# UnchartedWhispers/Distributed-Data-Parallel-Experiment

Measured on AMD Instinct MI355X. Metric: samples_per_sec_whole_node, higher is better.
Workload: dtype bf16

## Files before the change

### csrc/include/ddpx_wgrad_sgd.h

```cpp
#pragma once

#include <cstdlib>

#include "ddpx_mx.h"
#include "ddpx_pipe.h"

namespace ddpx {
namespace wsgd {

constexpr int BM = 64, BN = 128;
constexpr int A_SUB = BM * 64 * 2, B_SUB = BN * 64 * 2, SLOT = A_SUB + B_SUB;
constexpr int VPT = BM * BN / 4 / 256;
constexpr int kStampSlots = 256;

template <int STAGES>
struct Cfg {
  static_assert(STAGES == 3 || STAGES == 4, "ring depth");
  static constexpr int ALD = STAGES >= 4 ? BN : BN + 4;
  static constexpr int ACC_BYTES = BM * ALD * 4;
  static constexpr int LDS_BYTES = STAGES * SLOT + 2 * ACC_BYTES;
  static_assert(LDS_BYTES <= 160 * 1024, "LDS");
};

template <int STAGES, bool FP8, int NSW, bool NORD, int NMW, int PROBE = 0>
__global__ void __launch_bounds__(64 * NMW + 64 * NSW) wgrad_sgd_ws_kernel(pipe::Params p0, pipe::Params p1, int nt1) {
  constexpr int ALD = Cfg<STAGES>::ALD, ACC_BYTES = Cfg<STAGES>::ACC_BYTES;
  constexpr int LDS_BYTES = Cfg<STAGES>::LDS_BYTES;
  static_assert(NMW == 4 || NMW == 8, "math waves");
  static_assert(PROBE == 0 || PROBE == 3 || PROBE == 4, "probe");
  constexpr int WN = NMW / 2;
  constexpr int FM = 2, FN = BN / WN / 16;
  constexpr int LPW = (BM + BN) / (8 * NMW);
  __shared__ __attribute__((aligned(1024))) char smem[LDS_BYTES];
  float* const accb = reinterpret_cast<float*>(smem + STAGES * SLOT);

  const int tid = threadIdx.x;
  const int lane = tid & 63;
  const int wave = __builtin_amdgcn_readfirstlane(tid >> 6);
  const int tiles_m0 = p0.M / BM, tiles_m1 = p1.M / BM;
  const int nt0 = tiles_m0 * (p0.N / BN);
  const int ntiles = nt0 + nt1;
  const int nt = (ntiles - (int)blockIdx.x + (int)gridDim.x - 1) / (int)gridDim.x;
  const int nk = p0.K / 64;
  auto tile_origin = [&](int i, int& m0, int& n0) -> int {
    int g = (int)blockIdx.x + i * (int)gridDim.x;
    const int sel = g >= nt0;
    if (sel) g -= nt0;
    if constexpr (NORD) {
      const int tn = (sel ? p1.N : p0.N) / BN;
      m0 = (g / tn) * BM;
      n0 = (g % tn) * BN;
    } else {
      const int tm = sel ? tiles_m1 : tiles_m0;
      m0 = (g % tm) * BM;
      n0 = (g / tm) * BN;
    }
    return sel;
  };
  const pipe::Params& p = p0;
  long long* const stp = (p0.stamp && (tid == 0 || tid == 64 * NMW))
                             ? p0.stamp + ((size_t)blockIdx.x * 2 + (wave < NMW ? 0 : 1)) * kStampSlots
                             : nullptr;
  int nstamp = 1;
  auto mark = [&]() {
    if (stp) {
      stp[nstamp < kStampSlots - 1 ? nstamp : kStampSlots - 2] = (long long)__builtin_amdgcn_s_memrealtime();
      ++nstamp;
    }
  };
  if (stp) stp[0] = (long long)__builtin_amdgcn_s_memrealtime();

  if (wave < NMW) {
    const int wm = wave / WN, wn = wave % WN;
    const __amdgpu_buffer_rsrc_t ra0 = __builtin_amdgcn_make_buffer_rsrc((void*)p0.A, 0, p0.a_bytes, 0x00020000);
    const __amdgpu_buffer_rsrc_t rb0 = __builtin_amdgcn_make_buffer_rsrc((void*)p0.B, 0, p0.b_bytes, 0x00020000);
    const __amdgpu_buffer_rsrc_t ra1 = __builtin_amdgcn_make_buffer_rsrc((void*)p1.A, 0, p1.a_bytes, 0x00020000);
    const __amdgpu_buffer_rsrc_t rb1 = __builtin_amdgcn_make_buffer_rsrc((void*)p1.B, 0, p1.b_bytes, 0x00020000);
    const int G = nt * nk;
    int iss_i = -1, iss_kt = nk - 1, iss_m0 = 0, iss_n0 = 0, iss_sel = 0;
    auto issue = [&](int g) {
      if constexpr (PROBE == 4) return;
      if (++iss_kt >= nk) {
        iss_kt = 0;
        iss_sel = tile_origin(++iss_i, iss_m0, iss_n0);
      }
      const int m0 = iss_m0, n0 = iss_n0, sel = iss_sel, kt = iss_kt;
      const __amdgpu_buffer_rsrc_t ra = sel ? ra1 : ra0, rb = sel ? rb1 : rb0;
      const int lda = sel ? p1.lda : p0.lda, ldb = sel ? p1.ldb : p0.ldb;
      const int Mg = sel ? p1.M : p0.M, Ng = sel ? p1.N : p0.N;
      char* slot = smem + (g % STAGES) * SLOT;
      pipe::stage_tile<BM, false, pipe::MODE_PLAIN, NMW>(ra, slot, p.conv, lda, m0, Mg, kt * 64, p.K, wave, lane);
      pipe::stage_tile<BN, false, pipe::MODE_PLAIN, NMW>(rb, slot + A_SUB, p.conv, ldb, n0, Ng, kt * 64, p.K, wave,
                                                         lane);
    };
#pragma unroll
    for (int s = 0; s < STAGES - 1; ++s)
      if (s < G) issue(s);
    for (int i = 0; i <= nt; ++i) {
      if (i == nt) {
        for (int t = 0; t < nk; ++t) {
          mark();
          __builtin_amdgcn_s_barrier();
        }
      } else {
        f32x4 acc[FM][FN];
#pragma unroll
        for (int a = 0; a < FM; ++a)
#pragma unroll
          for (int b = 0; b < FN; ++b) acc[a][b] = (f32x4){0.f, 0.f, 0.f, 0.f};
        for (int t = 0; t < nk; ++t) {
          const int g = i * nk + t;
          const int ahead = min(STAGES - 2, G - 1 - g);
          if (STAGES >= 4 && ahead >= 2) pipe::wait_vmcnt<2 * LPW>();
          else if (ahead >= 1) pipe::wait_vmcnt<LPW>();
          else pipe::wait_vmcnt<0>();
          mark();
          __builtin_amdgcn_s_barrier();
          asm volatile("" ::: "memory");
          if (g + STAGES - 1 < G) issue(g + STAGES - 1);
          const char* sa = smem + (g % STAGES) * SLOT;
          const char* sb = sa + A_SUB;
#pragma unroll
          for (int kk = 0; kk < (PROBE == 4 ? 0 : 64); kk += 32) {
            bf16x8 af[FM], bfr[FN];
            pipe::load_frags<BM, false, FM, BN, false, FN>(sa, wm * 32, sb, wn * (BN / WN), kk, lane, af, bfr);
#pragma unroll
            for (int a = 0; a < FM; ++a)
#pragma unroll
              for (int b = 0; b < FN; ++b)
                acc[a][b] = __builtin_amdgcn_mfma_f32_16x16x32_bf16(af[a], bfr[b], acc[a][b], 0, 0, 0);
          }
        }
        float* T = accb + (i & 1) * (ACC_BYTES / 4);
        const int mr = wm * 32 + 4 * (lane >> 4), nc = wn * (BN / WN) + (lane & 15);
#pragma unroll
        for (int a = 0; a < FM; ++a)
#pragma unroll
          for (int b = 0; b < FN; ++b)
#pragma unroll
            for (int r = 0; r < 4; ++r) T[(mr + a * 16 + r) * ALD + nc + b * 16] = acc[a][b][r] * p.alpha;
      }
      asm volatile("s_waitcnt lgkmcnt(0)" ::: "memory");
      mark();
      __builtin_amdgcn_s_barrier();
    }
    if (stp) stp[kStampSlots - 1] = (long long)__builtin_amdgcn_s_memrealtime();
  } else {
    constexpr int DIST = 4;
    constexpr int SV = BM * BN / 4 / (NSW * 64);
    constexpr int KPU = VPT / SV;
    constexpr int RSTEP = NSW * 2;
    static_assert(SV % DIST == 0 && VPT % SV == 0, "ring");
    const int st = tid - 64 * NMW;
    const int row0 = st >> 5, col = 4 * (st & 31);
    const float lr = *p.sgd.lr;
    const float mom = p.sgd.mom, wd = p.sgd.wd;
    const bool has_mom = mom != 0.f;
    f32x4 rp[DIST], rm[DIST];
    float* const P0 = p0.sgd.p;
    float* const P1 = p1.sgd.p;
    float* const M0 = has_mom ? p0.sgd.buf : p0.sgd.p;
    float* const M1 = has_mom ? p1.sgd.buf : p1.sgd.p;
    unsigned short* const S0 = p0.sgd.shadow;
    unsigned short* const S1 = p1.sgd.shadow;
    unsigned char* const Q0 = p0.sgd.q8;
    unsigned char* const Q1 = p1.sgd.q8;
    unsigned char* const E0 = p0.sgd.s8;
    unsigned char* const E1 = p1.sgd.s8;
    unsigned char* const QT0 = p0.sgd.q8t;
    unsigned char* const QT1 = p1.sgd.q8t;
    unsigned char* const ET0 = p0.sgd.s8t;
    unsigned char* const ET1 = p1.sgd.s8t;
    const bool qt_on = FP8 && NSW == 8 && (QT0 != nullptr || QT1 != nullptr);
    unsigned qt_e0 = 0;
    const int ldc0 = p0.ldc, ldc1 = p1.ldc;
    auto vec_off = [&](int j, int v, int& sel) -> size_t {
      int m0, n0;
      sel = tile_origin(j, m0, n0);
      return (size_t)(m0 + row0 + RSTEP * v) * (sel ? ldc1 : ldc0) + n0 + col;
    };
    auto load_vec = [&](int j, int v, f32x4& pv, f32x4& mv) {
      int sel;
      const size_t off = vec_off(j, v, sel);
      pv = __builtin_nontemporal_load(reinterpret_cast<const f32x4*>((sel ? P1 : P0) + off));
      mv = __builtin_nontemporal_load(reinterpret_cast<const f32x4*>((sel ? M1 : M0) + off));
    };
    auto grad_vec = [&](const float* T, int v) -> f32x4 {
      return *reinterpret_cast<const f32x4*>(T + (row0 + RSTEP * v) * ALD + col);
    };
    auto update_vec_g = [&](int j, int v, const f32x4 g, f32x4& pv, f32x4& mv, float* stage) {
      int sel;
      const size_t off = vec_off(j, v, sel);
      f32x4 po, bo;
#pragma unroll
      for (int q = 0; q < 4; ++q) {
        float d = fmaf(wd, pv[q], g[q]);
        if (has_mom) d = fmaf(mom, mv[q], d);
        po[q] = fmaf(-lr, d, pv[q]);
        bo[q] = has_mom ? d : po[q];
      }
      if (stage) *reinterpret_cast<f32x4*>(stage) = po;
      const u32x2 sh = (u32x2){pack_bf2(po[0], po[1]), pack_bf2(po[2], po[3])};
      __builtin_nontemporal_store(po, reinterpret_cast<f32x4*>((sel ? P1 : P0) + off));
      __builtin_nontemporal_store(bo, reinterpret_cast<f32x4*>((sel ? M1 : M0) + off));
      *reinterpret_cast<u32x2*>((sel ? S1 : S0) + off) = sh;
      if constexpr (FP8) {
        unsigned e8;
        const unsigned q = mx::e4m3_group8(po, &e8);
        *reinterpret_cast<unsigned*>((sel ? Q1 : Q0) + off) = q;
        const unsigned e1 = (unsigned)__builtin_amdgcn_update_dpp(0, (int)e8, 0x128, 0xF, 0xF, false);
        if ((lane & 15) == 0)
          *reinterpret_cast<unsigned short*>((sel ? E1 : E0) + (off >> 5)) = (unsigned short)(e8 | (e1 << 8));
      }
      const int vn = v + DIST;
      const bool same = vn < SV, next = !same && j + 1 < nt;
      load_vec(same ? j : (next ? j + 1 : j), same ? vn : (next ? vn - SV : v), pv, mv);
    };
    auto update_vec = [&](int j, int v, const float* T, f32x4& pv, f32x4& mv) {
      if constexpr (FP8 && NSW == 8) {
        if (qt_on) {
          float* slot = const_cast<float*>(T) + (row0 + RSTEP * v) * ALD + col;
          const f32x4 g = *reinterpret_cast<const f32x4*>(slot);
          update_vec_g(j, v, g, pv, mv, slot);
          asm volatile("s_waitcnt lgkmcnt(0)" ::: "memory");
          return;
        }
      }
      update_vec_g(j, v, grad_vec(T, v), pv, mv, nullptr);
    };
    auto quant_t = [&](int j, int b, const float* T) {
      int m0, n0;
      const int sel = tile_origin(j, m0, n0);
      unsigned char* const qd = sel ? QT1 : QT0;
      if (!qd) return;
      const int c = st >> 2, sub = st & 3;
      float v[8];
      float am = 0.f;
#pragma unroll
      for (int r = 0; r < 8; ++r) {
        v[r] = bf2f(f2bf(T[(32 * b + 8 * sub + r) * ALD + c]));
        am = fmaxf(am, fabsf(v[r]));
      }
      am = fmaxf(am, __builtin_bit_cast(float, __builtin_amdgcn_update_dpp(0, __builtin_bit_cast(int, am), 0xB1, 0xF, 0xF, false)));
      am = fmaxf(am, __builtin_bit_cast(float, __builtin_amdgcn_update_dpp(0, __builtin_bit_cast(int, am), 0x4E, 0xF, 0xF, false)));
      const int e = mx::block_exp(am, mx::kMaxE4M3);
      const float inv = ldexpf(1.f, -e);
      const unsigned lo = mx::quant4(v[0], v[1], v[2], v[3], inv, mx::kMaxE4M3, false);
      const unsigned hi = mx::quant4(v[4], v[5], v[6], v[7], inv, mx::kMaxE4M3, false);
      const int Mg = sel ? p1.M : p0.M;
      *reinterpret_cast<u32x2*>(qd + (size_t)(n0 + c) * Mg + m0 + 32 * b + 8 * sub) = (u32x2){lo, hi};
      unsigned char* const ed = sel ? ET1 : ET0;
      if (sub == 0 && ed) {
        if (b == 0) {
          qt_e0 = (unsigned)(e + 127);
        } else {
          *reinterpret_cast<unsigned short*>(ed + (size_t)(n0 + c) * (Mg / 32) + m0 / 32) =
              (unsigned short)(qt_e0 | ((unsigned)(e + 127) << 8));
        }
      }
    };
#pragma unroll
    for (int v = 0; v < DIST; ++v)
      if constexpr (PROBE != 3) load_vec(0, v, rp[v], rm[v]);
    for (int t = 0; t < nk; ++t) {
      mark();
      __builtin_amdgcn_s_barrier();
    }
    mark();
    __builtin_amdgcn_s_barrier();
    constexpr int TPI = SV / DIST;
    auto trip = [&](int r) {
      const int i = 1 + r / TPI, t = (r % TPI) * DIST;
      const float* T = accb + ((i - 1) & 1) * (ACC_BYTES / 4);
#pragma unroll
      for (int u = 0; u < DIST; ++u) {
        mark();
        __builtin_amdgcn_s_barrier();
        __builtin_amdgcn_sched_barrier(0);
        if constexpr (PROBE != 3) update_vec(i - 1, t + u, T, rp[u], rm[u]);
        __builtin_amdgcn_sched_barrier(0);
#pragma unroll
        for (int k = 1; k < KPU; ++k) {
          mark();
          __builtin_amdgcn_s_barrier();
        }
        if constexpr (FP8 && NSW == 8) {
          if (qt_on && (t + u) % 2 == 1) {
            quant_t(i - 1, (t + u) / 2, T);
            asm volatile("s_waitcnt lgkmcnt(0)" ::: "memory");
          }
        }
      }
      if (r % TPI == TPI - 1) {
        asm volatile("s_waitcnt lgkmcnt(0)" ::: "memory");
        mark();
        __builtin_amdgcn_s_barrier();
      }
    };
    trip(0);
#pragma unroll 1
    for (int r = 1; r < TPI * nt; ++r) trip(r);
    if (stp) stp[kStampSlots - 1] = (long long)__builtin_amdgcn_s_memrealtime();
  }
}

static inline bool eligible(const pipe::Params& p, bool ak, bool bk) {
  return !ak && !bk && p.M % BM == 0 && p.N % BN == 0 && p.K == 64 * VPT && (p.ldc & 3) == 0 && p.sgd.p &&
         p.sgd.lr && (p.sgd.mom == 0.f || p.sgd.buf) && p.sgd.shadow && (!p.sgd.q8 || (p.sgd.s8 && (p.ldc & 127) == 0 && !((uintptr_t)p.sgd.q8 & 3) && !((uintptr_t)p.sgd.s8 & 3))) &&
         (!p.sgd.q8t || (p.sgd.q8 && !((uintptr_t)p.sgd.q8t & 7) && !((uintptr_t)p.sgd.s8t & 1)));
}

struct Variant {
  int stages;
  bool fp8;
  int nsw;
  bool nord;
  int nmw;
  int probe;
};

static inline int env_digit(const char* name) {
  const char* e = getenv(name);
  return e && e[0] >= '0' && e[0] <= '9' ? e[0] - '0' : -1;
}

static inline Variant select_variant(long long ntiles, int num_cus, bool fp8, bool qt) {
  static const int env_stages = env_digit("DDPX_WSGD_STAGES"), env_nsw = env_digit("DDPX_WSGD_STREAM_WAVES");
  static const int env_nmw = env_digit("DDPX_WSGD_MATH_WAVES");
  static const int env_probe = [] {
    const char* e = getenv("DDPX_WSGD_XTRA");
    return e ? atoi(e) : 0;
  }();
  static const bool env_nord = [] {
    const char* e = getenv("DDPX_WSGD_ORDER");
    return !(e && e[0] == 'm');
  }();
  const bool large = ntiles >= 64LL * num_cus;
  Variant v;
  v.stages = (env_stages == 3 || env_stages == 4) ? env_stages : (large ? 4 : 3);
  v.fp8 = fp8;
  v.nsw = qt ? 8 : (env_nsw == 4 || env_nsw == 8) ? env_nsw : (large ? 8 : 4);
  v.nord = env_nord;
  v.nmw = (env_nmw != 4 && v.nsw == 4 && v.nord) ? 8 : 4;
  const bool toy = !fp8 && v.stages == 3 && v.nsw == 4 && v.nord;
  v.probe = (toy && (env_probe == 3 || env_probe == 4)) ? env_probe : 0;
  return v;
}

using Kernel = void (*)(pipe::Params, pipe::Params, int);

template <int STAGES, bool FP8>
static inline Kernel layout_kernel(const Variant& v) {
  if (v.nmw == 8) return wgrad_sgd_ws_kernel<STAGES, FP8, 4, true, 8>;
  if (v.nsw == 8) return v.nord ? wgrad_sgd_ws_kernel<STAGES, FP8, 8, true, 4>
                                : wgrad_sgd_ws_kernel<STAGES, FP8, 8, false, 4>;
  return v.nord ? wgrad_sgd_ws_kernel<STAGES, FP8, 4, true, 4> : wgrad_sgd_ws_kernel<STAGES, FP8, 4, false, 4>;
}

static inline Kernel kernel_of(const Variant& v) {
  if (v.probe == 3)
    return v.nmw == 8 ? wgrad_sgd_ws_kernel<3, false, 4, true, 8, 3> : wgrad_sgd_ws_kernel<3, false, 4, true, 4, 3>;
  if (v.probe == 4)
    return v.nmw == 8 ? wgrad_sgd_ws_kernel<3, false, 4, true, 8, 4> : wgrad_sgd_ws_kernel<3, false, 4, true, 4, 4>;
  if (v.stages == 4) return v.fp8 ? layout_kernel<4, true>(v) : layout_kernel<4, false>(v);
  return v.fp8 ? layout_kernel<3, true>(v) : layout_kernel<3, false>(v);
}

static inline hipError_t launch_variant(const pipe::Params& p0, const pipe::Params& p1, int nt1, bool qt, int num_cus,
                                        hipStream_t s) {
  const int ntiles = (p0.M / BM) * (p0.N / BN) + nt1;
  const int grid = ntiles < num_cus ? ntiles : num_cus;
  const Variant v = select_variant(ntiles, num_cus, p0.sgd.q8 != nullptr, qt);
  hipLaunchKernelGGL(kernel_of(v), dim3(grid), dim3(64 * (v.nmw + v.nsw)), 0, s, p0, p1, nt1);
  return hipGetLastError();
}

static inline hipError_t launch(const pipe::Params& p, int num_cus, hipStream_t s) {
  return launch_variant(p, p, 0, false, num_cus, s);
}

static inline bool pair_compatible(const pipe::Params& a, const pipe::Params& b) {
  return a.K == b.K && a.alpha == b.alpha && a.sgd.lr == b.sgd.lr && a.sgd.mom == b.sgd.mom && a.sgd.wd == b.sgd.wd;
}

static inline hipError_t launch_pair(const pipe::Params& p0, const pipe::Params& p1, int num_cus, hipStream_t s) {
  if ((p0.sgd.q8 != nullptr) != (p1.sgd.q8 != nullptr)) return hipErrorInvalidValue;
  const bool qt = p0.sgd.q8t != nullptr || p1.sgd.q8t != nullptr;
  if (qt && !p0.sgd.q8) return hipErrorInvalidValue;
  return launch_variant(p0, p1, (p1.M / BM) * (p1.N / BN), qt, num_cus, s);
}

}
}
```

### csrc/kernels/gemm_pipe.hip

```cpp
#include <cstdlib>

#include "ddpx_gemm_dispatch.h"
#include "ddpx_pipe.h"
#include "ddpx_wgrad_sgd.h"

namespace ddpx {
namespace pipe {

static int pick(int M, int N, int K, bool ak, bool bk) {
  auto tiles = [&](int bm, int bn) { return ((M + bm - 1) / bm) * ((N + bn - 1) / bn); };
  if (!ak && !bk) return tiles(64, 128) >= 512 ? 5 : 7;
  if (tiles(128, 128) >= 512 && K >= 2048) return 21;
  return 12;
}

static int plan(int M, int N, int K, bool ak, bool bk, int epi, int* cfg) {
  *cfg = pick(M, N, K, ak, bk);
  static const int sk_cfg = [] {
    const char* e = getenv("DDPX_SPLITK");
    return e ? atoi(e) : 0;
  }();
  static const int sk_max = [] {
    const char* e = getenv("DDPX_SPLITK_MAX");
    return e ? atoi(e) : 2;
  }();
  if (sk_cfg <= 0 || !ak || epi == EPI_SGD || epi == EPI_BNSTAT_BF16 || K < 1024) return 1;
  int bm, bn;
  tile_of(sk_cfg, &bm, &bn);
  const int target = (sk_cfg == 5 || sk_cfg == 6 || sk_cfg == 7) ? 512 : 256;
  const int t = ((M + bm - 1) / bm) * ((N + bn - 1) / bn);
  if (t * 4 >= target * 3) return 1;
  int s = target / t;
  if (s > sk_max) s = sk_max;
  while (s > 1 && (K / 64) / s < 8) --s;
  if (s < 2) return 1;
  *cfg = sk_cfg;
  return s;
}

}
}

using namespace ddpx;

static long long* g_stamp = nullptr;

DDPX_API void ddpx_gemm_set_stamps(long long* buf) { g_stamp = buf; }

DDPX_API int ddpx_gemm_pipe_tiles_m(int M, int N, int K, int a_kcontig, int b_kcontig, int tile_cfg) {
  int cfg = tile_cfg;
  if (cfg < 0) pipe::plan(M, N, K, a_kcontig, b_kcontig, pipe::EPI_BF16, &cfg);
  int bm, bn;
  pipe::tile_of(cfg, &bm, &bn);
  return (M + bm - 1) / bm;
}

DDPX_API void ddpx_gemm_tile_dims(int cfg, int* bm, int* bn) { pipe::tile_of(cfg, bm, bn); }

DDPX_API int ddpx_gemm_pipe_plan(int M, int N, int K, int a_kcontig, int b_kcontig, int epi, int* cfg,
                                 long long* slab_floats, int* tickets) {
  const int s = pipe::plan(M, N, K, a_kcontig, b_kcontig, epi, cfg);
  int bm, bn;
  pipe::tile_of(*cfg, &bm, &bn);
  const long long tiles = (long long)((M + bm - 1) / bm) * ((N + bn - 1) / bn);
  *slab_floats = s > 1 ? (long long)s * tiles * bm * bn : 0;
  *tickets = s > 1 ? (int)tiles : 0;
  return s;
}

DDPX_API int ddpx_gemm_pipe(const void* A, const void* B, void* C, const float* bias, const void* aux, float* colsum,
                            int M, int N, int K, int lda, int ldb, int ldc, int ldaux, int a_kcontig, int b_kcontig,
                            int epi, int accumulate, float alpha, int tile_cfg, float* sgd_p, float* sgd_buf,
                            void* sgd_shadow, const float* sgd_lr, float sgd_mom, float sgd_wd, int splits,
                            float* slab, long long slab_floats, int* tcnt, void* cs_out, int cs_flags,
                            int* cs_tcnt, hipStream_t stream) {
  if (M <= 0 || N <= 0 || K <= 0) return 0;
  if (a_kcontig ? (K % 8 || lda % 8) : (M % 8 || lda % 8)) return -1;
  if (b_kcontig ? (K % 8 || ldb % 8) : (N % 8 || ldb % 8)) return -2;
  if ((reinterpret_cast<uintptr_t>(A) | reinterpret_cast<uintptr_t>(B)) & 15) return -3;
  const size_t a_bytes = (size_t)(a_kcontig ? (size_t)(M - 1) * lda + K : (size_t)(K - 1) * lda + M) * 2;
  const size_t b_bytes = (size_t)(b_kcontig ? (size_t)(N - 1) * ldb + K : (size_t)(K - 1) * ldb + N) * 2;
  if (a_bytes >= 0x80000000ull || b_bytes >= 0x80000000ull) return -4;
  pipe::Params p{(const unsigned short*)A, (const unsigned short*)B, C, bias, (const unsigned short*)aux, colsum,
                 M, N, K, lda, ldb, ldc, ldaux, epi, accumulate, alpha, (unsigned)a_bytes, (unsigned)b_bytes,
                 SgdArgs{sgd_p, sgd_buf, (unsigned short*)sgd_shadow, sgd_lr, sgd_mom, sgd_wd},
                 pipe::make_geom(0, 0, 0, 0), 0, 0, 0, nullptr, 0u, nullptr, cs_out, cs_flags, cs_tcnt};
  p.stamp = g_stamp;
  if (cs_tcnt && (!colsum || epi == pipe::EPI_SGD || epi == pipe::EPI_BNSTAT_BF16 || (!cs_out && !sgd_p) ||
                  (sgd_p && !sgd_lr)))
    return -10;
  if (epi == pipe::EPI_SGD && (!sgd_p || !sgd_lr || (sgd_mom != 0.f && !sgd_buf))) return -5;
  static const int sgd_plain = [] {
    const char* e = getenv("DDPX_SGD_PLAIN");
    return e && e[0] == '1' ? 1 : 0;
  }();
  p.sgd_plain = sgd_plain;
  int cfg = tile_cfg >= 0 ? tile_cfg : pipe::pick(M, N, K, a_kcontig, b_kcontig);
  if (cs_tcnt && pipe::eight_wave(cfg)) return -11;
  if (cfg >= 16 && cfg <= 20 && (epi == pipe::EPI_SGD || epi == pipe::EPI_BNSTAT_BF16)) return -12;
  if (splits > 1) {
    if (epi == pipe::EPI_SGD || epi == pipe::EPI_BNSTAT_BF16 || !slab || !tcnt || tile_cfg < 0 || !a_kcontig)
      return -7;
    int bm, bn;
    pipe::tile_of(cfg, &bm, &bn);
    const long long tiles = (long long)((M + bm - 1) / bm) * ((N + bn - 1) / bn);
    if (slab_floats < (long long)splits * tiles * bm * bn || slab_floats * 4 >= 0x80000000ll) return -8;
    int klen = (K + splits - 1) / splits;
    klen = (klen + 63) / 64 * 64;
    if ((K + klen - 1) / klen != splits) return -9;
    p.klen = klen;
    p.slab = slab;
    p.slab_bytes = (unsigned)(slab_floats * 4);
    p.tcnt = tcnt;
  }
  if (tile_cfg < 0 && !a_kcontig && !b_kcontig && epi != pipe::EPI_SGD && !colsum &&
      ((M + 255) / 256) * ((N + 255) / 256) >= 128)
    cfg = 13;
  static const int wgrad_ws = [] {
    const char* e = getenv("DDPX_WGRAD_WS");
    return e && e[0] == '0' ? 0 : 1;
  }();
  if (epi == pipe::EPI_SGD && wgrad_ws && tile_cfg < 0 && splits <= 1 && wsgd::eligible(p, a_kcontig, b_kcontig)) {
    static const int cus = [] {
      int dev = 0, n = 0;
      if (hipGetDevice(&dev) != hipSuccess ||
          hipDeviceGetAttribute(&n, hipDeviceAttributeMultiprocessorCount, dev) != hipSuccess || n <= 0)
        n = 256;
      return n;
    }();
    return (int)wsgd::launch(p, cus, stream);
  }
  hipError_t e;
  if (splits > 1) {
    e = b_kcontig ? pipe::dispatch_sk_kk(p, cfg, splits, stream) : pipe::dispatch_sk_kn(p, cfg, splits, stream);
    return (int)e;
  }
  const int S = 1;
  if (a_kcontig && b_kcontig) e = pipe::dispatch_kk(p, cfg, S, stream);
  else if (a_kcontig) e = pipe::dispatch_kn(p, cfg, S, stream);
  else if (b_kcontig) e = pipe::dispatch_mk(p, cfg, S, stream);
  else e = pipe::dispatch_mn(p, cfg, S, stream);
  return (int)e;
}

DDPX_API int ddpx_wgrad_sgd_pair_t(const void* A0, const void* B0, int M0, int N0, int lda0, int ldb0, int ldc0,
                                   float* p0, float* buf0, void* sh0, void* q80, void* s80, void* q8t0, void* s8t0,
                                   const void* A1, const void* B1, int M1, int N1, int lda1, int ldb1, int ldc1,
                                   float* p1, float* buf1, void* sh1, void* q81, void* s81, void* q8t1, void* s8t1,
                                   int K, const float* lr, float mom, float wd, hipStream_t stream) {
  auto make = [&](const void* A, const void* B, int M, int N, int lda, int ldb, int ldc, float* pp, float* buf,
                  void* sh, void* q8, void* s8, void* q8t, void* s8t) {
    const size_t a_bytes = ((size_t)(K - 1) * lda + M) * 2, b_bytes = ((size_t)(K - 1) * ldb + N) * 2;
    return pipe::Params{(const unsigned short*)A, (const unsigned short*)B, pp, nullptr, nullptr, nullptr,
                        M, N, K, lda, ldb, ldc, 0, pipe::EPI_SGD, 0, 1.f, (unsigned)a_bytes, (unsigned)b_bytes,
                        SgdArgs{pp, buf, (unsigned short*)sh, lr, mom, wd, (unsigned char*)q8, (unsigned char*)s8,
                                (unsigned char*)q8t, (unsigned char*)s8t},
                        pipe::make_geom(0, 0, 0, 0), 0, 0, 0, nullptr, 0u, nullptr, nullptr, 0, nullptr};
  };
  if (K <= 0 || lda0 % 8 || ldb0 % 8 || lda1 % 8 || ldb1 % 8 || M0 % 8 || N0 % 8 || M1 % 8 || N1 % 8) return -20;
  if (((uintptr_t)A0 | (uintptr_t)B0 | (uintptr_t)A1 | (uintptr_t)B1) & 15) return -20;
  if ((q8t0 || q8t1) && (!q80 || !q81)) return -20;
  pipe::Params q0 = make(A0, B0, M0, N0, lda0, ldb0, ldc0, p0, buf0, sh0, q80, s80, q8t0, s8t0);
  const pipe::Params q1 = make(A1, B1, M1, N1, lda1, ldb1, ldc1, p1, buf1, sh1, q81, s81, q8t1, s8t1);
  q0.stamp = g_stamp;
  if ((size_t)q0.a_bytes != ((size_t)(K - 1) * lda0 + M0) * 2 || (size_t)q1.b_bytes != ((size_t)(K - 1) * ldb1 + N1) * 2)
    return -20;
  if (!wsgd::eligible(q0, false, false) || !wsgd::eligible(q1, false, false) || !wsgd::pair_compatible(q0, q1))
    return -20;
  if ((q80 != nullptr) != (q81 != nullptr)) return -20;
  int dev = 0, cus = 0;
  if (hipGetDevice(&dev) != hipSuccess ||
      hipDeviceGetAttribute(&cus, hipDeviceAttributeMultiprocessorCount, dev) != hipSuccess || cus <= 0)
    cus = 256;
  return (int)wsgd::launch_pair(q0, q1, cus, stream);
}

DDPX_API int ddpx_wgrad_sgd_pair(const void* A0, const void* B0, int M0, int N0, int lda0, int ldb0, int ldc0,
                                 float* p0, float* buf0, void* sh0, void* q80, void* s80, const void* A1,
                                 const void* B1, int M1, int N1, int lda1, int ldb1, int ldc1, float* p1, float* buf1,
                                 void* sh1, void* q81, void* s81, int K, const float* lr, float mom, float wd,
                                 hipStream_t stream) {
  return ddpx_wgrad_sgd_pair_t(A0, B0, M0, N0, lda0, ldb0, ldc0, p0, buf0, sh0, q80, s80, nullptr, nullptr, A1, B1,
                               M1, N1, lda1, ldb1, ldc1, p1, buf1, sh1, q81, s81, nullptr, nullptr, K, lr, mom, wd,
                               stream);
}
```

### ddpx/ops/gemm.py

```python
from __future__ import annotations

import torch

from ..runtime import native


EPI_F32 = 0
EPI_BF16 = 1
EPI_BIAS_BF16 = 2
EPI_BIAS_RELU_BF16 = 3
EPI_BIAS_F32 = 4
EPI_RELUMASK_BF16 = 5
EPI_SGD = 6

_OUT_DTYPE = {
    EPI_F32: torch.float32,
    EPI_BF16: torch.bfloat16,
    EPI_BIAS_BF16: torch.bfloat16,
    EPI_BIAS_RELU_BF16: torch.bfloat16,
    EPI_BIAS_F32: torch.float32,
    EPI_RELUMASK_BF16: torch.bfloat16,
}


def _req(cond, msg):
    if not cond:
        raise ValueError(msg)


def _check_bf16_2d(t, name):
    _req(t.is_cuda, f"{name} must be a GPU tensor")
    _req(t.dtype == torch.bfloat16, f"{name} must be bf16, got {t.dtype}")
    _req(t.dim() == 2, f"{name} must be 2-D, got shape {tuple(t.shape)}")
    _req(t.stride(1) == 1, f"{name} must be row-contiguous")
    _req(t.stride(0) % 8 == 0, f"{name} leading dimension must be a multiple of 8")
    _req(t.data_ptr() % 16 == 0, f"{name} must be 16-byte aligned")


def plan(M, N, K, a_kcontig, b_kcontig, epi):
    cfg = native.c_int(0)
    sf = native.c_int64(0)
    nt = native.c_int(0)
    s = native.kernels().ddpx_gemm_pipe_plan(M, N, K, int(a_kcontig), int(b_kcontig), int(epi),
                                             native.ctypes.byref(cfg), native.ctypes.byref(sf), native.ctypes.byref(nt))
    return s, cfg.value, sf.value, nt.value


_TICKETS: dict = {}
_CS_TICKETS: dict = {}
_RETIRED: list = []


def _tickets(dev, n, pool=None):
    pool = _TICKETS if pool is None else pool
    t = pool.get(dev)
    if t is None or t.numel() < n:
        if torch.cuda.is_current_stream_capturing():
            raise RuntimeError("GEMM tickets: first launch of this size must happen outside graph capture")
        if t is not None:
            _RETIRED.append(t)
        t = pool[dev] = torch.zeros((max(n, 4096),), dtype=torch.int32, device=dev)
    return t


def tile_dims(cfg):
    bm, bn = native.c_int(0), native.c_int(0)
    native.kernels().ddpx_gemm_tile_dims(int(cfg), native.ctypes.byref(bm), native.ctypes.byref(bn))
    return bm.value, bn.value


def gemm_raw(a, b, c, *, M, N, K, lda, ldb, ldc, a_kcontig, b_kcontig, epi, bias=None, aux=None, ldaux=0,
             accumulate=False, alpha=1.0, tile=-1, colsum=None, stream=None, sgd=None, splits=None,
             cs_out=None, cs_accumulate=False, cs_sgd=None):
    lib = native.kernels()
    s = native.stream_handle(stream)
    slab, sf, tk = None, 0, None
    nt = 0
    if splits is not None and splits > 1:
        _req(tile >= 0 and sgd is None, "forced split-K needs an explicit tile and no fused optimizer")
        bm, bn = tile_dims(tile)
        nt = ((M + bm - 1) // bm) * ((N + bn - 1) // bn)
        sf = splits * nt * bm * bn
    else:
        splits = 1
        if tile < 0 and sgd is None:
            splits, cfg, sf, nt = plan(M, N, K, a_kcontig, b_kcontig, epi)
            if splits > 1:
                tile = cfg
    if splits > 1:
        slab = torch.empty(sf, dtype=torch.float32, device=a.device)
        tk = _tickets(a.device, nt)
    cs_t, cs_flags = None, 0
    if cs_out is not None or cs_sgd is not None:
        _req(colsum is not None and sgd is None, "in-launch column sums need the colsum scratch, no EPI_SGD")
        cs_t = _tickets(a.device, N, pool=_CS_TICKETS)
        cs_flags = int(cs_out is not None and cs_out.dtype == torch.bfloat16) | (2 if cs_accumulate else 0)
        sgd = cs_sgd
    rc = lib.ddpx_gemm_pipe(a.data_ptr(), b.data_ptr(), c.data_ptr(), native.ptr(bias), native.ptr(aux),
                            native.ptr(colsum), M, N, K, lda, ldb, ldc, ldaux, int(a_kcontig), int(b_kcontig), epi,
                            int(accumulate), float(alpha), tile, *native.sgd_args(sgd), splits, native.ptr(slab), sf,
                            native.ptr(tk), native.ptr(cs_out), cs_flags, native.ptr(cs_t), s)
    native.check(rc, f"ddpx_gemm_pipe(M={M},N={N},K={K},epi={epi})")
    return c


def tiles_m(M, N, K, a_kcontig, b_kcontig, tile=-1):
    return native.kernels().ddpx_gemm_pipe_tiles_m(M, N, K, int(a_kcontig), int(b_kcontig), tile)


def linear_fwd(x, w, bias=None, relu=False, out=None, out_dtype=torch.bfloat16, tile=-1, splits=None):
    _check_bf16_2d(x, "x")
    _check_bf16_2d(w, "w")
    M, K = x.shape
    N, K2 = w.shape
    _req(K == K2, f"inner dims differ: x {tuple(x.shape)} vs w {tuple(w.shape)}")
    if bias is not None:
        _req(bias.dtype == torch.float32 and bias.numel() == N and bias.is_contiguous(), "bias must be fp32 [N]")
    if out_dtype == torch.bfloat16:
        epi = EPI_BIAS_RELU_BF16 if relu else (EPI_BIAS_BF16 if bias is not None else EPI_BF16)
        _req(not (relu and bias is None), "relu epilogue requires a bias")
    else:
        _req(not relu, "fp32 output epilogue has no relu")
        epi = EPI_BIAS_F32 if bias is not None else EPI_F32
    if out is None:
        out = torch.empty((M, N), dtype=_OUT_DTYPE[epi], device=x.device)
    _req(tuple(out.shape) == (M, N) and out.stride(1) == 1 and out.stride(0) % 8 == 0
         and out.data_ptr() % 16 == 0 and out.dtype == _OUT_DTYPE[epi], "bad out tensor")
    return gemm_raw(x, w, out, M=M, N=N, K=K, lda=x.stride(0), ldb=w.stride(0), ldc=out.stride(0), a_kcontig=True,
                    b_kcontig=True, epi=epi, bias=bias, tile=tile, splits=splits)


def linear_dgrad(dy, w, relu_mask_of=None, out=None, tile=-1, bias_grad=None, bias_grad_accumulate=False,
                 bias_sgd=None, splits=None):
    _check_bf16_2d(dy, "dy")
    _check_bf16_2d(w, "w")
    M, N = dy.shape
    N2, K = w.shape
    _req(N == N2, f"dy {tuple(dy.shape)} incompatible with w {tuple(w.shape)}")
    epi = EPI_BF16
    if relu_mask_of is not None:
        _check_bf16_2d(relu_mask_of, "relu_mask_of")
        _req(tuple(relu_mask_of.shape) == (M, K), "mask shape must equal dX shape")
        epi = EPI_RELUMASK_BF16
    if out is None:
        out = torch.empty((M, K), dtype=torch.bfloat16, device=dy.device)
    _req(out.shape == (M, K) and out.is_contiguous() and out.dtype == torch.bfloat16, "bad out tensor")
    part = None
    if bias_grad is not None or bias_sgd is not None:
        _req(bias_grad is None or (bias_grad.numel() == K and bias_grad.is_contiguous()),
             "bias_grad must be contiguous [K]")
        _req(bias_sgd is None or bias_sgd[0].numel() == K, "bias_sgd target must have K elements")
        T = tiles_m(M, K, N, True, False, tile)
        part = torch.empty((T, K), dtype=torch.float32, device=dy.device)
    in_launch = tile not in _EIGHT_WAVE_TILES
    _req(in_launch or bias_sgd is None, "fused bias SGD needs a 4-wave dgrad tile")
    gemm_raw(dy, w, out, M=M, N=K, K=N, lda=dy.stride(0), ldb=w.stride(0), ldc=K, a_kcontig=True,
             b_kcontig=False, epi=epi, aux=relu_mask_of,
             ldaux=(relu_mask_of.stride(0) if relu_mask_of is not None else 0), tile=tile, colsum=part,
             splits=splits,
             cs_out=bias_grad if in_launch else None, cs_accumulate=bias_grad_accumulate,
             cs_sgd=bias_sgd if in_launch else None)
    if part is not None and not in_launch and bias_grad is not None:
        s = part.sum(0).to(bias_grad.dtype)
        bias_grad.add_(s) if bias_grad_accumulate else bias_grad.copy_(s)
    return out


_EIGHT_WAVE_TILES = (8, 13, 14, 15, 22, 25)


def linear_wgrad(dy, x, out, accumulate=False, tile=-1, sgd=None):
    if sgd is not None:
        _check_bf16_2d(dy, "dy")
        _check_bf16_2d(x, "x")
        M, N = dy.shape
        _, K = x.shape
        _req(sgd[0].numel() == N * K, "sgd target size mismatch")
        return gemm_raw(dy, x, sgd[0], M=N, N=K, K=M, lda=dy.stride(0), ldb=x.stride(0), ldc=K, a_kcontig=False,
                        b_kcontig=False, epi=EPI_SGD, tile=tile, sgd=sgd)
    _check_bf16_2d(dy, "dy")
    _check_bf16_2d(x, "x")
    M, N = dy.shape
    M2, K = x.shape
    _req(M == M2, f"batch dims differ: dy {tuple(dy.shape)} vs x {tuple(x.shape)}")
    _req(out.dtype in (torch.float32, torch.bfloat16), "dW must be fp32 or bf16")
    _req(tuple(out.shape) == (N, K) and out.is_contiguous(), f"dW must be contiguous [{N},{K}]")
    epi = EPI_F32 if out.dtype == torch.float32 else EPI_BF16
    return gemm_raw(dy, x, out, M=N, N=K, K=M, lda=dy.stride(0), ldb=x.stride(0), ldc=K, a_kcontig=False,
                    b_kcontig=False, epi=epi, accumulate=accumulate, tile=tile)


def matmul(a, b, a_kcontig=True, b_kcontig=True, out_dtype=torch.float32, tile=-1):
    _check_bf16_2d(a, "a")
    _check_bf16_2d(b, "b")
    M, K = a.shape if a_kcontig else (a.shape[1], a.shape[0])
    N, K2 = b.shape if b_kcontig else (b.shape[1], b.shape[0])
    _req(K == K2, "inner dims differ")
    epi = EPI_F32 if out_dtype == torch.float32 else EPI_BF16
    out = torch.empty((M, N), dtype=out_dtype, device=a.device)
    return gemm_raw(a, b, out, M=M, N=N, K=K, lda=a.stride(0), ldb=b.stride(0), ldc=N, a_kcontig=a_kcontig,
                    b_kcontig=b_kcontig, epi=epi, tile=tile)


native.register_kernel_sig("ddpx_wgrad_sgd_pair", native.c_int, *([native.c_void_p, native.c_void_p] + [native.c_int] * 5
                                                                  + [native.c_void_p] * 5) * 2,
                           native.c_int, native.c_void_p, native.c_float, native.c_float, native.c_void_p)


native.register_kernel_sig("ddpx_wgrad_sgd_pair_t", native.c_int, *([native.c_void_p, native.c_void_p] + [native.c_int] * 5
                                                                    + [native.c_void_p] * 7) * 2,
                           native.c_int, native.c_void_p, native.c_float, native.c_float, native.c_void_p)


def wgrad_sgd_pair(dy0, x0, sgd0, dy1, x1, sgd1, mx0=None, mx1=None, mxt0=None, mxt1=None) -> bool:
    for t, n in ((dy0, "dy0"), (x0, "x0"), (dy1, "dy1"), (x1, "x1")):
        _check_bf16_2d(t, n)
    if dy0.shape[0] != dy1.shape[0] or x0.shape[0] != dy0.shape[0] or x1.shape[0] != dy1.shape[0]:
        return False
    if sgd0[3] is not sgd1[3] or sgd0[4] != sgd1[4] or sgd0[5] != sgd1[5]:
        return False
    K = dy0.shape[0]
    transposed = mxt0 is not None or mxt1 is not None
    if transposed and (mx0 is None or mx1 is None):
        return False
    args = []
    for dy, x, sg, mx, mxt in ((dy0, x0, sgd0, mx0, mxt0), (dy1, x1, sgd1, mx1, mxt1)):
        M, N = dy.shape[1], x.shape[1]
        _req(sg[0].numel() == M * N, "sgd target size mismatch")
        if mx is not None:
            _req(mx[0].dtype == torch.uint8 and mx[0].numel() == M * N and mx[0].is_contiguous()
                 and mx[1].dtype == torch.uint8 and mx[1].numel() == M * N // 32 and N % 32 == 0,
                 "fp8 copy must be uint8 [M, N] codes + [M, N/32] scales")
        if mxt is not None:
            _req(mxt[0].dtype == torch.uint8 and tuple(mxt[0].shape) == (N, M) and mxt[0].is_contiguous()
                 and mxt[1].dtype == torch.uint8 and tuple(mxt[1].shape) == (N, M // 32) and mxt[1].is_contiguous()
                 and M % 64 == 0, "transposed fp8 copy must be uint8 [N, M] codes + [N, M/32] scales, M % 64 == 0")
        args += [dy.data_ptr(), x.data_ptr(), M, N, dy.stride(0), x.stride(0), N, sg[0].data_ptr(),
                 native.ptr(sg[1]), native.ptr(sg[2]), native.ptr(mx[0] if mx else None),
                 native.ptr(mx[1] if mx else None)]
        if transposed:
            args += [native.ptr(mxt[0] if mxt else None), native.ptr(mxt[1] if mxt else None)]
    lr = sg[3]
    fn = native.kernels().ddpx_wgrad_sgd_pair_t if transposed else native.kernels().ddpx_wgrad_sgd_pair
    rc = fn(*args, K, lr.data_ptr(), float(sgd0[4]), float(sgd0[5]), native.stream_handle())
    if rc == -20:
        return False
    native.check(rc, "ddpx_wgrad_sgd_pair")
    return True
```

Baseline: 2.291 million.

## Add 128-row tile variant with single swizzled accumulator buffer to fused wgrad-SGD

Adds a BM=128 tile option for the warp-specialized wgrad+SGD kernel, using 8 math waves and a single XOR-swizzled LDS accumulator buffer instead of double buffering. The stream waves read gradients from LDS ahead of the barrier. A 128-row tile is chosen automatically when there are enough tiles and the shapes allow it. The intent is more MFMA reuse per loaded B tile and fewer tiles to schedule. The cost is extra synchronization on the shared accumulator, plus a new plan query entry point.

Result: faster. 2.459 million, median of 6 (+7.3%).

```diff
diff --git a/csrc/include/ddpx_wgrad_sgd.h b/csrc/include/ddpx_wgrad_sgd.h
--- a/csrc/include/ddpx_wgrad_sgd.h
+++ b/csrc/include/ddpx_wgrad_sgd.h
@@ -8,28 +8,37 @@
 namespace ddpx {
 namespace wsgd {
 
-constexpr int BM = 64, BN = 128;
-constexpr int A_SUB = BM * 64 * 2, B_SUB = BN * 64 * 2, SLOT = A_SUB + B_SUB;
-constexpr int VPT = BM * BN / 4 / 256;
+constexpr int BN = 128;
+constexpr int NK = 8;
 constexpr int kStampSlots = 256;
 
-template <int STAGES>
+template <int BM, int STAGES>
 struct Cfg {
-  static_assert(STAGES == 3 || STAGES == 4, "ring depth");
-  static constexpr int ALD = STAGES >= 4 ? BN : BN + 4;
+  static_assert(BM == 64 || BM == 128, "tile height");
+  static_assert(STAGES == 3 || (STAGES == 4 && BM == 64), "ring depth");
+  static constexpr int A_SUB = BM * 64 * 2, B_SUB = BN * 64 * 2, SLOT = A_SUB + B_SUB;
+  static constexpr bool SBUF = BM == 128;
+  static constexpr int ALD = (STAGES >= 4 || SBUF) ? BN : BN + 4;
   static constexpr int ACC_BYTES = BM * ALD * 4;
-  static constexpr int LDS_BYTES = STAGES * SLOT + 2 * ACC_BYTES;
+  static constexpr int LDS_BYTES = STAGES * SLOT + (SBUF ? 1 : 2) * ACC_BYTES;
   static_assert(LDS_BYTES <= 160 * 1024, "LDS");
+  __host__ __device__ static constexpr int tile_col(int row, int col) {
+    return SBUF ? (col ^ (((row >> 2) & 3) << 4)) : col;
+  }
 };
 
-template <int STAGES, bool FP8, int NSW, bool NORD, int NMW, int PROBE = 0>
+template <int BM, int STAGES, bool FP8, int NSW, bool NORD, int NMW, int PROBE = 0>
 __global__ void __launch_bounds__(64 * NMW + 64 * NSW) wgrad_sgd_ws_kernel(pipe::Params p0, pipe::Params p1, int nt1) {
-  constexpr int ALD = Cfg<STAGES>::ALD, ACC_BYTES = Cfg<STAGES>::ACC_BYTES;
-  constexpr int LDS_BYTES = Cfg<STAGES>::LDS_BYTES;
+  using C = Cfg<BM, STAGES>;
+  constexpr int ALD = C::ALD, ACC_BYTES = C::ACC_BYTES, LDS_BYTES = C::LDS_BYTES;
+  constexpr int A_SUB = C::A_SUB, SLOT = C::SLOT;
+  constexpr bool SBUF = C::SBUF;
   static_assert(NMW == 4 || NMW == 8, "math waves");
+  static_assert(BM == 64 || (NMW == 8 && !FP8), "the 128-row tile: 8 math waves, no MX-FP8 copy");
   static_assert(PROBE == 0 || PROBE == 3 || PROBE == 4, "probe");
   constexpr int WN = NMW / 2;
-  constexpr int FM = 2, FN = BN / WN / 16;
+  constexpr int WMR = BM / 2;
+  constexpr int FM = WMR / 16, FN = BN / WN / 16;
   constexpr int LPW = (BM + BN) / (8 * NMW);
   __shared__ __attribute__((aligned(1024))) char smem[LDS_BYTES];
   float* const accb = reinterpret_cast<float*>(smem + STAGES * SLOT);
@@ -41,7 +50,7 @@
   const int nt0 = tiles_m0 * (p0.N / BN);
   const int ntiles = nt0 + nt1;
   const int nt = (ntiles - (int)blockIdx.x + (int)gridDim.x - 1) / (int)gridDim.x;
-  const int nk = p0.K / 64;
+  constexpr int nk = NK;
   auto tile_origin = [&](int i, int& m0, int& n0) -> int {
     int g = (int)blockIdx.x + i * (int)gridDim.x;
     const int sel = g >= nt0;
@@ -123,7 +132,7 @@
 #pragma unroll
           for (int kk = 0; kk < (PROBE == 4 ? 0 : 64); kk += 32) {
             bf16x8 af[FM], bfr[FN];
-            pipe::load_frags<BM, false, FM, BN, false, FN>(sa, wm * 32, sb, wn * (BN / WN), kk, lane, af, bfr);
+            pipe::load_frags<BM, false, FM, BN, false, FN>(sa, wm * WMR, sb, wn * (BN / WN), kk, lane, af, bfr);
 #pragma unroll
             for (int a = 0; a < FM; ++a)
 #pragma unroll
@@ -131,14 +140,17 @@
                 acc[a][b] = __builtin_amdgcn_mfma_f32_16x16x32_bf16(af[a], bfr[b], acc[a][b], 0, 0, 0);
           }
         }
-        float* T = accb + (i & 1) * (ACC_BYTES / 4);
-        const int mr = wm * 32 + 4 * (lane >> 4), nc = wn * (BN / WN) + (lane & 15);
+        float* T = accb + (SBUF ? 0 : (i & 1) * (ACC_BYTES / 4));
+        const int mr = wm * WMR + 4 * (lane >> 4), nc = wn * (BN / WN) + (lane & 15);
 #pragma unroll
         for (int a = 0; a < FM; ++a)
 #pragma unroll
           for (int b = 0; b < FN; ++b)
 #pragma unroll
-            for (int r = 0; r < 4; ++r) T[(mr + a * 16 + r) * ALD + nc + b * 16] = acc[a][b][r] * p.alpha;
+            for (int r = 0; r < 4; ++r) {
+              const int row = mr + a * 16 + r;
+              T[row * ALD + C::tile_col(row, nc + b * 16)] = acc[a][b][r] * p.alpha;
+            }
       }
       asm volatile("s_waitcnt lgkmcnt(0)" ::: "memory");
       mark();
@@ -148,9 +160,11 @@
   } else {
     constexpr int DIST = 4;
     constexpr int SV = BM * BN / 4 / (NSW * 64);
-    constexpr int KPU = VPT / SV;
+    constexpr int UPK = SV >= NK ? SV / NK : 1;
+    constexpr int KPU = SV >= NK ? 1 : NK / SV;
     constexpr int RSTEP = NSW * 2;
-    static_assert(SV % DIST == 0 && VPT % SV == 0, "ring");
+    static_assert(SV % DIST == 0 && DIST % UPK == 0 && SV * KPU == NK * UPK, "ring");
+    static_assert(!SBUF || KPU == 1, "single buffer: at least one update per K-step");
     const int st = tid - 64 * NMW;
     const int row0 = st >> 5, col = 4 * (st & 31);
     const float lr = *p.sgd.lr;
@@ -186,7 +200,8 @@
       mv = __builtin_nontemporal_load(reinterpret_cast<const f32x4*>((sel ? M1 : M0) + off));
     };
     auto grad_vec = [&](const float* T, int v) -> f32x4 {
-      return *reinterpret_cast<const f32x4*>(T + (row0 + RSTEP * v) * ALD + col);
+      const int row = row0 + RSTEP * v;
+      return *reinterpret_cast<const f32x4*>(T + row * ALD + C::tile_col(row, col));
     };
     auto update_vec_g = [&](int j, int v, const f32x4 g, f32x4& pv, f32x4& mv, float* stage) {
       int sel;
@@ -269,15 +284,35 @@
     mark();
     __builtin_amdgcn_s_barrier();
     constexpr int TPI = SV / DIST;
+    f32x4 gq[UPK];
+    auto read_ahead = [&](int v0) {
+      if constexpr (SBUF && PROBE != 3) {
+#pragma unroll
+        for (int k = 0; k < UPK; ++k) gq[k] = grad_vec(accb, v0 + k);
+      }
+    };
+    read_ahead(0);
     auto trip = [&](int r) {
       const int i = 1 + r / TPI, t = (r % TPI) * DIST;
-      const float* T = accb + ((i - 1) & 1) * (ACC_BYTES / 4);
+      const float* T = accb + (SBUF ? 0 : ((i - 1) & 1) * (ACC_BYTES / 4));
+      f32x4 gc[UPK];
 #pragma unroll
       for (int u = 0; u < DIST; ++u) {
-        mark();
-        __builtin_amdgcn_s_barrier();
-        __builtin_amdgcn_sched_barrier(0);
-        if constexpr (PROBE != 3) update_vec(i - 1, t + u, T, rp[u], rm[u]);
+        if (u % UPK == 0) {
+          if constexpr (SBUF) asm volatile("s_waitcnt lgkmcnt(0)" ::: "memory");
+          mark();
+          __builtin_amdgcn_s_barrier();
+          __builtin_amdgcn_sched_barrier(0);
+          if constexpr (SBUF && PROBE != 3) {
+#pragma unroll
+            for (int k = 0; k < UPK; ++k) gc[k] = gq[k];
+            if (u + UPK < DIST || r % TPI != TPI - 1) read_ahead(t + u + UPK);
+          }
+        }
+        if constexpr (PROBE != 3) {
+          if constexpr (SBUF) update_vec_g(i - 1, t + u, gc[u % UPK], rp[u], rm[u], nullptr);
+          else update_vec(i - 1, t + u, T, rp[u], rm[u]);
+        }
         __builtin_amdgcn_sched_barrier(0);
 #pragma unroll
         for (int k = 1; k < KPU; ++k) {
@@ -295,6 +330,7 @@
         asm volatile("s_waitcnt lgkmcnt(0)" ::: "memory");
         mark();
         __builtin_amdgcn_s_barrier();
+        read_ahead(0);
       }
     };
     trip(0);
@@ -305,12 +341,13 @@
 }
 
 static inline bool eligible(const pipe::Params& p, bool ak, bool bk) {
-  return !ak && !bk && p.M % BM == 0 && p.N % BN == 0 && p.K == 64 * VPT && (p.ldc & 3) == 0 && p.sgd.p &&
+  return !ak && !bk && p.M % 64 == 0 && p.N % BN == 0 && p.K == 64 * NK && (p.ldc & 3) == 0 && p.sgd.p &&
          p.sgd.lr && (p.sgd.mom == 0.f || p.sgd.buf) && p.sgd.shadow && (!p.sgd.q8 || (p.sgd.s8 && (p.ldc & 127) == 0 && !((uintptr_t)p.sgd.q8 & 3) && !((uintptr_t)p.sgd.s8 & 3))) &&
          (!p.sgd.q8t || (p.sgd.q8 && !((uintptr_t)p.sgd.q8t & 7) && !((uintptr_t)p.sgd.s8t & 1)));
 }
 
 struct Variant {
+  int bm;
   int stages;
   bool fp8;
   int nsw;
@@ -324,11 +361,15 @@
   return e && e[0] >= '0' && e[0] <= '9' ? e[0] - '0' : -1;
 }
 
-static inline Variant select_variant(long long ntiles, int num_cus, bool fp8, bool qt) {
+static inline Variant select_variant(long long ntiles, int num_cus, bool fp8, bool qt, bool m128) {
   static const int env_stages = env_digit("DDPX_WSGD_STAGES"), env_nsw = env_digit("DDPX_WSGD_STREAM_WAVES");
   static const int env_nmw = env_digit("DDPX_WSGD_MATH_WAVES");
   static const int env_probe = [] {
     const char* e = getenv("DDPX_WSGD_XTRA");
+    return e ? atoi(e) : 0;
+  }();
+  static const int env_tile = [] {
+    const char* e = getenv("DDPX_WSGD_TILE");
     return e ? atoi(e) : 0;
   }();
   static const bool env_nord = [] {
@@ -337,11 +378,15 @@
   }();
   const bool large = ntiles >= 64LL * num_cus;
   Variant v;
+  v.bm = 64;
   v.stages = (env_stages == 3 || env_stages == 4) ? env_stages : (large ? 4 : 3);
   v.fp8 = fp8;
   v.nsw = qt ? 8 : (env_nsw == 4 || env_nsw == 8) ? env_nsw : (large ? 8 : 4);
   v.nord = env_nord;
   v.nmw = (env_nmw != 4 && v.nsw == 4 && v.nord) ? 8 : 4;
+  const bool can128 = m128 && !fp8 && !qt && env_stages != 4 && env_nsw != 8 && env_nmw != 4 && env_nord;
+  const bool want128 = env_tile == 128 || (env_tile != 64 && ntiles >= 2LL * num_cus);
+  if (want128 && can128) v.bm = 128, v.stages = 3, v.nsw = 4, v.nmw = 8;
   const bool toy = !fp8 && v.stages == 3 && v.nsw == 4 && v.nord;
   v.probe = (toy && (env_probe == 3 || env_probe == 4)) ? env_probe : 0;
   return v;
@@ -351,32 +396,44 @@
 
 template <int STAGES, bool FP8>
 static inline Kernel layout_kernel(const Variant& v) {
-  if (v.nmw == 8) return wgrad_sgd_ws_kernel<STAGES, FP8, 4, true, 8>;
-  if (v.nsw == 8) return v.nord ? wgrad_sgd_ws_kernel<STAGES, FP8, 8, true, 4>
-                                : wgrad_sgd_ws_kernel<STAGES, FP8, 8, false, 4>;
-  return v.nord ? wgrad_sgd_ws_kernel<STAGES, FP8, 4, true, 4> : wgrad_sgd_ws_kernel<STAGES, FP8, 4, false, 4>;
+  if (v.nmw == 8) return wgrad_sgd_ws_kernel<64, STAGES, FP8, 4, true, 8>;
+  if (v.nsw == 8) return v.nord ? wgrad_sgd_ws_kernel<64, STAGES, FP8, 8, true, 4>
+                                : wgrad_sgd_ws_kernel<64, STAGES, FP8, 8, false, 4>;
+  return v.nord ? wgrad_sgd_ws_kernel<64, STAGES, FP8, 4, true, 4> : wgrad_sgd_ws_kernel<64, STAGES, FP8, 4, false, 4>;
 }
 
 static inline Kernel kernel_of(const Variant& v) {
+  if (v.bm == 128) {
+    if (v.probe == 3) return wgrad_sgd_ws_kernel<128, 3, false, 4, true, 8, 3>;
+    if (v.probe == 4) return wgrad_sgd_ws_kernel<128, 3, false, 4, true, 8, 4>;
+    return wgrad_sgd_ws_kernel<128, 3, false, 4, true, 8>;
+  }
   if (v.probe == 3)
-    return v.nmw == 8 ? wgrad_sgd_ws_kernel<3, false, 4, true, 8, 3> : wgrad_sgd_ws_kernel<3, false, 4, true, 4, 3>;
+    return v.nmw == 8 ? wgrad_sgd_ws_kernel<64, 3, false, 4, true, 8, 3> : wgrad_sgd_ws_kernel<64, 3, false, 4, true, 4, 3>;
   if (v.probe == 4)
-    return v.nmw == 8 ? wgrad_sgd_ws_kernel<3, false, 4, true, 8, 4> : wgrad_sgd_ws_kernel<3, false, 4, true, 4, 4>;
+    return v.nmw == 8 ? wgrad_sgd_ws_kernel<64, 3, false, 4, true, 8, 4> : wgrad_sgd_ws_kernel<64, 3, false, 4, true, 4, 4>;
   if (v.stages == 4) return v.fp8 ? layout_kernel<4, true>(v) : layout_kernel<4, false>(v);
   return v.fp8 ? layout_kernel<3, true>(v) : layout_kernel<3, false>(v);
 }
 
-static inline hipError_t launch_variant(const pipe::Params& p0, const pipe::Params& p1, int nt1, bool qt, int num_cus,
-                                        hipStream_t s) {
-  const int ntiles = (p0.M / BM) * (p0.N / BN) + nt1;
+static inline Variant plan(const pipe::Params& p0, const pipe::Params& p1, bool pair, bool qt, int num_cus) {
+  const long long nt64 = (long long)(p0.M / 64) * (p0.N / BN) + (pair ? (long long)(p1.M / 64) * (p1.N / BN) : 0);
+  const bool m128 = p0.M % 128 == 0 && (!pair || p1.M % 128 == 0);
+  return select_variant(nt64, num_cus, p0.sgd.q8 != nullptr, qt, m128);
+}
+
+static inline hipError_t launch_variant(const pipe::Params& p0, const pipe::Params& p1, bool pair, bool qt,
+                                        int num_cus, hipStream_t s) {
+  const Variant v = plan(p0, p1, pair, qt, num_cus);
+  const int nt1 = pair ? (p1.M / v.bm) * (p1.N / BN) : 0;
+  const int ntiles = (p0.M / v.bm) * (p0.N / BN) + nt1;
   const int grid = ntiles < num_cus ? ntiles : num_cus;
-  const Variant v = select_variant(ntiles, num_cus, p0.sgd.q8 != nullptr, qt);
   hipLaunchKernelGGL(kernel_of(v), dim3(grid), dim3(64 * (v.nmw + v.nsw)), 0, s, p0, p1, nt1);
   return hipGetLastError();
 }
 
 static inline hipError_t launch(const pipe::Params& p, int num_cus, hipStream_t s) {
-  return launch_variant(p, p, 0, false, num_cus, s);
+  return launch_variant(p, p, false, false, num_cus, s);
 }
 
 static inline bool pair_compatible(const pipe::Params& a, const pipe::Params& b) {
@@ -387,8 +444,8 @@
   if ((p0.sgd.q8 != nullptr) != (p1.sgd.q8 != nullptr)) return hipErrorInvalidValue;
   const bool qt = p0.sgd.q8t != nullptr || p1.sgd.q8t != nullptr;
   if (qt && !p0.sgd.q8) return hipErrorInvalidValue;
-  return launch_variant(p0, p1, (p1.M / BM) * (p1.N / BN), qt, num_cus, s);
-}
-
-}
-}
+  return launch_variant(p0, p1, true, qt, num_cus, s);
+}
+
+}
+}
diff --git a/csrc/kernels/gemm_pipe.hip b/csrc/kernels/gemm_pipe.hip
--- a/csrc/kernels/gemm_pipe.hip
+++ b/csrc/kernels/gemm_pipe.hip
@@ -184,3 +184,25 @@
                                M1, N1, lda1, ldb1, ldc1, p1, buf1, sh1, q81, s81, nullptr, nullptr, K, lr, mom, wd,
                                stream);
 }
+
+DDPX_API int ddpx_wgrad_sgd_plan(int M0, int N0, int M1, int N1, int K, int fp8, int qt, int* bm, int* stages,
+                                 int* nsw, int* nmw) {
+  const bool pair = M1 > 0;
+  auto shape_ok = [&](int M, int N) { return M > 0 && N > 0 && M % 64 == 0 && N % wsgd::BN == 0; };
+  if (K != 64 * wsgd::NK || !shape_ok(M0, N0) || (pair && !shape_ok(M1, N1)) || (qt && !fp8)) return -20;
+  pipe::Params q0{}, q1{};
+  q0.M = M0, q0.N = N0, q0.K = K;
+  q1.M = pair ? M1 : M0, q1.N = pair ? N1 : N0, q1.K = K;
+  static unsigned char fp8_mark;
+  if (fp8) q0.sgd.q8 = q1.sgd.q8 = &fp8_mark;
+  int dev = 0, cus = 0;
+  if (hipGetDevice(&dev) != hipSuccess ||
+      hipDeviceGetAttribute(&cus, hipDeviceAttributeMultiprocessorCount, dev) != hipSuccess || cus <= 0)
+    cus = 256;
+  const wsgd::Variant v = wsgd::plan(q0, q1, pair, qt != 0, cus);
+  if (bm) *bm = v.bm;
+  if (stages) *stages = v.stages;
+  if (nsw) *nsw = v.nsw;
+  if (nmw) *nmw = v.nmw;
+  return 0;
+}
diff --git a/ddpx/ops/gemm.py b/ddpx/ops/gemm.py
--- a/ddpx/ops/gemm.py
+++ b/ddpx/ops/gemm.py
@@ -212,6 +212,20 @@
                            native.c_int, native.c_void_p, native.c_float, native.c_float, native.c_void_p)
 
 
+native.register_kernel_sig("ddpx_wgrad_sgd_plan", native.c_int, *([native.c_int] * 7 + [native.c_void_p] * 4))
+
+
+def wgrad_sgd_plan(M0, N0, M1=0, N1=0, K=512, fp8=False, transposed=False):
+    import ctypes
+    out = [ctypes.c_int(0) for _ in range(4)]
+    rc = native.kernels().ddpx_wgrad_sgd_plan(int(M0), int(N0), int(M1), int(N1), int(K), int(bool(fp8)),
+                                              int(bool(transposed)), *[ctypes.addressof(o) for o in out])
+    if rc == -20:
+        return None
+    native.check(rc, "ddpx_wgrad_sgd_plan")
+    return dict(zip(("bm", "stages", "nsw", "nmw"), (o.value for o in out)))
+
+
 def wgrad_sgd_pair(dy0, x0, sgd0, dy1, x1, sgd1, mx0=None, mx1=None, mxt0=None, mxt1=None) -> bool:
     for t, n in ((dy0, "dy0"), (x0, "x0"), (dy1, "dy1"), (x1, "x1")):
         _check_bf16_2d(t, n)
```
